# mike-gimelfarb/bboptpy

Hardware: AMD Instinct MI355X
Metric: candidate-evals/sec (higher is better)
Workload: dtype f64; 1 GPU; ActiveCMAES n=128 np=4096 rosenbrock, 256 independent populations per GPU in lockstep; populations_per_gpu=256, n=128, np=4096, objective=rosenbrock

## Files before the change

bboptpy_amd/csrc/bbo_cma.hip:

```cpp
#include "bbo_cma_kernels.hpp"
#include "bbo_sep_kernels.hpp"
#include "bbo_chol_kernels.hpp"
#include "bbo_eig_mw.hpp"

#include <algorithm>
#include <atomic>
#include <cmath>
#include <cstdlib>
#include <limits>

namespace bbo {

namespace {

enum { K_SAMPLE = 0, K_RANK, K_WHITEN, K_GRAM, K_PATHS, K_COV, K_EIGEN, K_POST, K_STOP, K_COUNT };
static const char *const K_NAMES[K_COUNT] = { "bbo:cma_sample_eval", "bbo:cma_rank", "bbo:cma_whiten", "bbo:cma_gram", "bbo:cma_paths", "bbo:cma_cov", "bbo:cma_eigen", "bbo:cma_post", "bbo:cma_history_stop" };

int pick_maxt(int ld)
{
    const int per_wave = ((ld >> 4) + 3) / 4;
    if (per_wave <= 1) return 1;
    if (per_wave <= 2) return 2;
    if (per_wave <= 4) return 4;
    return 8;
// ... 604 lines not shown
    return counter.fetch_add(1) & 7;
}

EigRoute CmaEngine::eig_route(bool spread_ok, bool fuse_ok) const
{
    const CmaConst &c = c_;
    const int dbg = d_.dbg;
    EigRoute r {};
    if (c.variant >= 2) return r;
    auto add = [&r](EigKernel k, int arg = 0) { r.step[r.count++] = EigRoute::Step { k, arg }; };
    const EigPlan pl_lds = eig_plan(c.n, c.ld);
    r.split = pl_lds.use_lds && pl_lds.threads == 512 && pl_lds.dc && c.npop <= split_maxp_
            && !(dbg & (DBG_QL | DBG_DC_NO_MERGES | DBG_DC_NO_LEAVES | DBG_TRED_L2 | DBG_EIG_ONE_WG));
    const EigPlan pl = r.split ? eig_plan_split(c.n, c.ld) : pl_lds;
    spread_ok = spread_ok && !mw_disabled_;
    const bool fixed_shape = c.n == 128 && c.ld == 128 && !d_.stamps
            && !(dbg & (DBG_EIG_IN_KERNEL | DBG_EIG_GENERIC128));
    bool big_spread = false, wy4_packs = false, fcols_closed = false;
    if (c.n <= 16 && c.n >= 2 && c.ld == 16 && !(dbg & DBG_NO_EIGEN_SMALL))
        add(EK_EIGEN_SMALL);
    else if (pl.threads < 512)
        add(pl.threads == 128 ? EK_EIGEN_128 : EK_EIGEN_256);
    else if (fixed_shape && c.npop > split_maxp_ && c.lazy_isc) {
        r.fixed = true;
        r.forms_c = fuse_ok && !(dbg & DBG_COV_UNFUSED);
        add(r.forms_c ? EK_EIGEN_FX128 : EK_EIGEN_FX128U);
    } else if (pl.use_lds)
        add(EK_EIGEN);
    else if (pl.hybrid && !(dbg & (DBG_QL | DBG_TRED_L2 | DBG_EIG_ONE_WG))) {
        if (r.split) {
            r.fixed = fixed_shape;
            add(r.fixed ? EK_EIGEN_R1_FX128 : EK_EIGEN_R1);
        } else if (spread_ok && !(dbg & DBG_TRED_ONE_WG)) {
            r.mw_workgroups = (long) c.npop * MW_G;
            const int istop = (dbg & DBG_TRED_ALL_SPREAD) ? 1 : 128;
            add(EK_TRED_MW, istop);
            if (istop > 1) add(EK_TRED_TAIL);
        } else
            add(EK_EIGEN_G1);
        add(EK_EIG_HALVES);
        if ((long) c.npop * 8 <= 256 && !(dbg & DBG_TOP_ONE_KERNEL)) {
// ... 58 lines not shown
    };
    timer_.begin(stream_, K_EIGEN);
    for (int i = 0; i < r.count; i++) {
        if (i == r.timed) {
            timer_.end(stream_);
            BBO_HIP(hipGetLastError());
        }
        const int arg = r.step[i].arg;
        switch (r.step[i].k) {
        case EK_EIGEN_SMALL:
            hipLaunchKernelGGL(cma_eigen_small, dim3((c.npop + 3) / 4), dim3(256), 0, stream_, d_, c_, 0, 1);
            break;
        case EK_EIGEN_128: per_matrix(cma_eigen_128, 128, pl, d_, c_, pl, 0); break;
        case EK_EIGEN_256: per_matrix(cma_eigen_256, 256, pl, d_, c_, pl, 0); break;
        case EK_EIGEN: per_matrix(cma_eigen, 512, pl, d_, c_, pl, 0); break;
        case EK_EIGEN_FX128: per_matrix(cma_eigen_fx128, 512, EIG_FX_PLAN, fa); break;
        case EK_EIGEN_FX128U: per_matrix(cma_eigen_fx128u, 512, EIG_FX_PLAN, fa); break;
        case EK_EIGEN_R1: per_matrix(cma_eigen_r1, 512, pl_lds, d_, c_, pl_lds, 0); break;
        case EK_EIGEN_R1_FX128: per_matrix(cma_eigen_r1_fx128, 512, EIG_FX_PLAN, fa); break;
        case EK_EIGEN_G1: per_matrix(cma_eigen_g1, 512, pl, d_, c_, pl, 0); break;
        case EK_TRED_MW:
            mw_launched_ = true;
            if (mw_buf_.count != (size_t) c.npop * MW_BUF_DOUBLES) mw_buf_.alloc((size_t) c.npop * MW_BUF_DOUBLES);
            hipLaunchKernelGGL(cma_tred_mw, dim3(8 * MW_G, c.npop), dim3(MW_T), 0, stream_, d_, c_, 0,
                    mw_buf_.p, ++mw_launch_, arg, mw_xcd_);
            break;
        case EK_TRED_TAIL: {
            const EigPlan plt = c.n > 256 ? eig_plan(256, 256) : pl;
            per_matrix(cma_tred_tail, 512, plt, d_, c_, plt, arg);
            break;
        }
        case EK_EIG_HALVES:
// ... 104 lines not shown
void CmaEngine::generation(bool honor_stop)
{
    if (small_fused_ok()) {
        launch_small(1, honor_stop);
        return;
    }
    small_fused_ = false;
    c_.honor_stop = honor_stop ? 1 : 0;
    launch_sample_eval();
    if (obj_.needs_host()) host_evaluate();
    else if (obj_.is_program()) program_evaluate();
    launch_rank();
    const EigRoute route = eig_route(true, true);
    launch_update(!route.forms_c);
    launch_eigen(route);
    launch_history_stop();
}

void CmaEngine::phase(int which)
{
    BBO_REQUIRE(inited_, "phase before init");
    BBO_HIP(hipSetDevice(params_.device));
    c_.honor_stop = 0;
    d_.mw_fault = mw_fault_from_env();
    switch (which) {
    case BBO_PHASE_SAMPLE_EVALUATE:
        launch_sample_eval();
        if (obj_.needs_host()) host_evaluate();
        else if (obj_.is_program()) program_evaluate();
        break;
    case BBO_PHASE_RANK: launch_rank(); break;
// ... 224 lines not shown
    if (k == "eig_stage") return o.one(s.eig_stage);
    if (k == "eig_mw_fail") return o.one(s.eig_mw_fail);
    if (k == "chol_repairs") {
        if (c.variant != 3) throw Error(BBO_ERR_KEY, "'chol_repairs' belongs to CholeskyCMAES");
        int r = 0;
        chol_repairs_.download(&r, 1, p);
        return o.one(r);
    }
    if (c.variant == 3 && k == "chol_tri") return o.one(chol_tri_ ? 1 : 0);
    if (c.variant == 3 && k == "stol") return o.one(c.stol);
    if (c.variant == 3 && k == "ranked") return o.one(c.ranked);
    if (k == "eig_mw_off") return o.one(mw_disabled_ ? 1 : 0);
    if (k == "eig_split_maxp") return o.one(split_maxp_);
    if (k == "eig_fixed128") return o.one(last_route_.fixed ? 1 : 0);
    if (k == "cov_fused") return o.one(last_route_.forms_c ? 1 : 0);
    if (k == "eig_route") {
        double ids[sizeof(last_route_.step) / sizeof(last_route_.step[0])];
        for (int i = 0; i < last_route_.count; i++) ids[i] = last_route_.step[i].k;
        return o.copy(ids, last_route_.count);
    }
    if (k == "rank_route") return o.one(last_rank_);
    if (k == "sample_route") return o.one(last_sample_.k);
    if (k == "sample_lean") return o.one(last_sample_.full);
    if (k == "update_route") {
        double ids[sizeof(last_update_.step) / sizeof(last_update_.step[0])];
        for (int i = 0; i < last_update_.count; i++) ids[i] = last_update_.step[i].k;
        return o.copy(ids, last_update_.count);
    }
    if (k == "small_fused") return o.one(small_fused_ ? 1 : 0);
    if (k == "splits") return o.one(c.splits);
// ... 187 lines not shown
```

bboptpy_amd/csrc/bbo_cma.hpp:

```cpp
#pragma once

#include "bbo_engine.hpp"

namespace bbo {

struct CmaScal {
    double sigma;
    double fbest, fworst;
    double pslen;
    double ybw[4];
    int ibw[4];
    int it, fev;
    int flag;
    int stop;
    int hsig;
    int eigenlastev, eigen_done;
    int hist_head, hist_len;
    int basis_ok;
    int eig_stage;
    int eig_mw_fail;
};

struct CmaConst {
    int n, ld;
// ... 35 lines not shown
    DBG_DC_LEAF16        = 32768,
    DBG_GRAM_NO_PACING   = 65536,
    DBG_PATHS_LAZY256    = 131072,
    DBG_RANK_BITONIC     = 262144,
    DBG_DC_LEAF_SINGLE   = 524288,
    DBG_SEP_ROWS_LDS     = 1048576,
    DBG_EIG_GENERIC128   = 2097152,
    DBG_EIG_ONE_WG       = 4194304,
    DBG_DC_WG_BARRIERS   = 8388608,
    DBG_TRED_ONE_WG      = 16777216,
    DBG_TOP_PART2        = 33554432,
    DBG_TOP_ONE_KERNEL   = 67108864,
    DBG_WY_PER_WAVE      = 134217728,
    DBG_SAMPLE_4WAVES    = 268435456,
    DBG_TRED_ALL_SPREAD  = 536870912,
    DBG_EIG_IN_KERNEL    = DBG_QL_NO_APPLY | DBG_QL | DBG_DC_NO_MERGES | DBG_DC_NO_LEAVES | DBG_TRED_L2
                           | DBG_STAMPS_HALVES | DBG_DC_ONE_LEVEL | DBG_DC_TWO_LEVELS | DBG_DC_LEAF16
                           | DBG_DC_LEAF_SINGLE | DBG_EIG_ONE_WG | DBG_DC_WG_BARRIERS,
};

struct CmaDev {
    double *X;
    double *f;
    int *rank;
    int *order;
    double *xmean, *xold, *pc, *ps;
    double *C;
    double *B;
    double *D;
    double *isc;
// ... 13 lines not shown
    const double *zinject;
    double *zrecord;
    CmaScal *scal;
    long long *stamps;
    int dbg;
    int mw_fault;
    int *mw_fail_host;
};

enum EigKernel : int {
    EK_EIGEN_SMALL = 0, EK_EIGEN_128, EK_EIGEN_256, EK_EIGEN, EK_EIGEN_FX128, EK_EIGEN_FX128U,
    EK_EIGEN_R1, EK_EIGEN_R1_FX128, EK_EIGEN_G1, EK_TRED_MW, EK_TRED_TAIL, EK_EIG_HALVES,
    EK_EIGEN_G2, EK_EIG_SECULAR, EK_EIG_LOWNER, EK_EIG_FCOLS, EK_EIGEN_G,
    EK_TRED_MW512, EK_TRED_MW_CHAIN, EK_EIGEN_B4, EK_EIGEN_B,
    EK_EIG_GEMM1, EK_EIG_GEMM, EK_EIG_WY4, EK_EIG_WY4_512, EK_EIG_WY,
    EK_POST, EK_POST_MFMA
};

struct EigRoute {
    struct Step {
        EigKernel k;
        int arg;
    };
    Step step[12];
    int count;
    int timed;
    bool split;
    bool post;
    bool fixed;
    bool forms_c;
    long mw_workgroups;
};

enum SampleKernel : int {
    SK_NONE = -1,
    SK_SEP_16 = 0, SK_SEP_64_512, SK_SEP_64_512_LEAN, SK_SEP_SUM, SK_SEP_SUM4, SK_SEP_64,
    SK_EVAL128, SK_EVAL128_TRI, SK_TILE8, SK_TILE8_TRI,
    SK_EVAL64_1_8, SK_EVAL64_1, SK_EVAL64_2,
    SK_TILE16, SK_EVAL_4, SK_EVAL_8
};

struct SampleRoute {
    SampleKernel k;
    int gx, gy, block;
    size_t lds;
// ... 114 lines not shown
```

bboptpy_amd/csrc/bbo_cma_kernels.hpp:

```cpp
#pragma once

#include "bbo_cma.hpp"
#include "bbo_objectives.hpp"
#include "bbo_rng.hpp"
#include "bbo_eig.hpp"
#include "bbo_rank.hpp"

namespace bbo {

typedef double d4_t __attribute__((ext_vector_type(4)));

#define BBO_INF (__builtin_huge_val())

__device__ inline void cma_draw_quad(const CmaDev &d, const CmaConst &c, int p, int row, int q,
        int gen, uint32_t sw, const double2 *tab, double (&z)[4])
{
    const int j0 = cma_quad_col0(q);
    z[0] = z[1] = z[2] = z[3] = 0.;
    if (row < c.lambda && j0 < c.n) {
        if (d.zinject) {
            const double *zi = d.zinject + ((size_t) p * c.lambda + row) * c.n;
#pragma unroll
            for (int i = 0; i < 4; i++)
                if (j0 + 4 * i < c.n) z[i] = zi[j0 + 4 * i];
// ... 1573 lines not shown
        const bool in = i < n && j < n;
        BDp[q] = in ? Bs[i * ldp + j] * Dv[j] : 0.;
    }
    if (mode == 2) {
        for (int q = q0 + tid; q < q1; q += 256) {
            const int t4 = q >> 6, l = q & 63;
            const int nt = t4 / KS, ks = t4 - nt * KS;
            const int i = nt * 16 + (l & 15), j = 4 * ks + (l >> 4);
            ISp[q] = (i < n && j < n) ? isc[(size_t) i * ld + j] : 0.;
        }
    }
}

__device__ __forceinline__ void history_stop_body(const CmaDev &d, const CmaConst &c, int p, int lane)
{
    CmaScal *sc = d.scal + p;
    if (pop_frozen(c, sc)) return;
    const int ld = c.ld, n = c.n;
    double *hb = d.hist_best + (size_t) p * c.hlen, *hk = d.hist_kth + (size_t) p * c.hlen;
    const double *f = d.f + (size_t) p * c.lambda_pad;
    const int *order = d.order + (size_t) p * c.lambda_pad;
    int it = sc->it;
    int head = sc->hist_head, len = sc->hist_len;
    double fbest = sc->fbest, fworst = sc->fworst;

    if (it < c.mit) {
        head = (head + 1) % c.hlen;
        if (lane == 0) {
            hb[head] = f[order[0]];
            hk[head] = f[order[c.ik]];
        }
        if (len < c.hlen) len++;
        wave_sync();
        if (len == c.hlen) {
            double lo = BBO_INF, hi = -BBO_INF;
            for (int k = lane; k < c.hlen; k += 64) {
                lo = fmin(lo, hb[k]);
                hi = fmax(hi, hb[k]);
            }
#pragma unroll
            for (int off = 32; off > 0; off >>= 1) {
                lo = fmin(lo, __shfl_xor(lo, off, 64));
                hi = fmax(hi, __shfl_xor(hi, off, 64));
            }
            fbest = lo;
            fworst = hi;
        }
    }
    it++;
    wave_sync();

    const double sigma = sc->sigma;
    const double *pc = d.pc + (size_t) p * ld, *xm = d.xmean + (size_t) p * ld;
    const double *C = d.C + (size_t) p * ld * ld, *B = d.B + (size_t) p * ld * ld;
    const double *D = d.D + (size_t) p * ld;
    int flag = 0;
    const int off = c.stop_off;
    if (it >= c.mit) {
        flag = 1;
    } else if (f[order[0]] <= c.ftarget) {
        flag = 10;
    } else if (!(off & 4) && it >= c.hlen && fworst - fbest < c.tol) {
        flag = 2;
    } else {
        if (!(off & 8) && len >= n) {
            int eq = 0;
            for (int i = lane; i < n; i += 64) {
                const int idx = (c.hlen + head - i) % c.hlen;
                eq += hb[idx] == hk[idx];
            }
#pragma unroll
            for (int off = 32; off > 0; off >>= 1) eq += __shfl_xor(eq, off, 64);
            if (3 * eq >= n) flag = 3;
        }
        const bool sep = c.variant == 2;
        if (!flag && !(off & 16)) {
            int bad = 0;
            for (int i = lane; i < n; i += 64) {
                const double sd = sep ? D[i] : sqrt(C[(size_t) i * ld + i]);
                bad |= (fmax(pc[i], sd) * sigma / c.sigma0 >= c.tol);
            }
            if (!__any(bad)) flag = 4;
        }
        if (!flag && !(off & 32) && sigma / c.sigma0 > 1.0e20 * D[n - 1]) flag = 5;
        if (!flag && !(off & 128) && D[n - 1] > 1.0e7 * D[0]) flag = 7;
        if (!flag && !(off & 256)) {
            const int iaxis = n - 1 - ((it - 1) % n);
            int moved = 0;
            if (sep) {
                moved = xm[iaxis] != xm[iaxis] + 0.1 * sigma * D[iaxis];
            } else {
                for (int i = lane; i < n; i += 64)
                    moved |= (xm[i] != xm[i] + 0.1 * sigma * D[iaxis] * B[(size_t) iaxis * ld + i]);
            }
            if (!__any(moved)) flag = 8;
        }
        if (!flag && !(off & 512)) {
            int stuck = 0;
            for (int i = lane; i < n; i += 64) {
                const double sd = sep ? D[i] : sqrt(C[(size_t) i * ld + i]);
                stuck |= (xm[i] == xm[i] + 0.2 * sigma * sd);
            }
            if (__any(stuck)) flag = 9;
        }
    }
    if (lane == 0) {
        sc->it = it;
        sc->hist_head = head;
        sc->hist_len = len;
        sc->fbest = fbest;
        sc->fworst = fworst;
        sc->flag = flag;
        if (flag) sc->stop = 1;
        else if (sc->fev >= c.mfev) sc->stop = 2;
    }
}

__global__ __launch_bounds__(64) void cma_history_stop(CmaDev d, CmaConst c)
{
    history_stop_body(d, c, blockIdx.x, threadIdx.x);
}

constexpr int SMALL_FUSED_MAXP = 512;

__host__ __device__ inline int small_state_doubles(const CmaConst &c)
{
    const int ld = c.ld, ld2 = ld * ld, lp = c.lambda_pad;
    return lp * ld
            + 2 * lp + lp
            + 5 * ld
// ... 228 lines not shown
```

bboptpy_amd/csrc/bbo_eig.hpp:

```cpp
#pragma once

#include <type_traits>

#include "bbo_cma.hpp"
#include "bbo_eig_ql.hpp"
#include "bbo_eig_dc.hpp"

namespace bbo {

typedef double d4_eig __attribute__((ext_vector_type(4)));

constexpr int EIG_THREADS = 512;
constexpr int EIG_NMAX = 512;

struct EigPlan {
    int threads;
    int use_lds;
    int reg_path;
    int dc;
    int hybrid;
    int lda;
    int rc;
    int vl;
    size_t lds_bytes;
// ... 149 lines not shown
    for (int a = 0; a < AMAX; a++)
#pragma unroll
        for (int b = 0; b < 8; b += 2) {
            acc0 = __builtin_fma(ur[a][b], a_[a][b], acc0);
            acc1 = __builtin_fma(ur[a][b + 1], a_[a][b + 1], acc1);
        }
    double acc = acc0 + acc1;
    acc = eig_quad_sum(acc);
    const double gq = -(acc / h);
#pragma unroll
    for (int a = 0; a < AMAX; a++)
#pragma unroll
        for (int b = 0; b < 8; b++) a_[a][b] = __builtin_fma(gq, ur[a][b], a_[a][b]);
}

template<int TT = EIG_THREADS>
__device__ inline void eig_tred_accum_reg128(const double *C, int ld, int n, const EigMat &As,
        double *dv, double *ev, double *uv, double *wv, double *gv, double *hvec, double *td,
        int tid, long long *stamps, double *qdst, int ldq, bool finish, bool accumulate = true)
{
    const int T = TT, lane = tid & 63;
    const int j = tid >> 2, q = tid & 3;
    double a_[4][8];
#pragma unroll
    for (int a = 0; a < 4; a++)
#pragma unroll
        for (int b = 0; b < 8; b++) {
            const int k = 32 * a + 8 * q + b;
            a_[a][b] = (j < n && k < n) ? C[(size_t) j * ld + k] : 0.;
        }
    for (int k = tid; k < 128; k += T) {
// ... 717 lines not shown
        wv[k] = 0.;
    }
    __syncthreads();
    const int lda = A.ld;
    for (int q = tid; q < n * n; q += T) {
        const int r = q / n, cidx = q - r * n;
        double v = 0.;
        if (cidx < r) v = r < 128 ? As(r, cidx) : A.a[(size_t) r * lda + cidx];
        Vout[q] = v;
    }
    __syncthreads();
    for (int k = tid; k < n; k += T) dv[k] = td[k];
    __syncthreads();
}

template<int TT>
__device__ inline void eig_cov_prologue128(const CmaDev &d, const CmaConst &c, const CmaScal *sc, int p,
        double *As, int tid)
{
    constexpr int N = 128, LB = eig_plan(128, 128).lda, EPT = 12;
    double *C = d.C + (size_t) p * N * N;
    const int lane = tid & 63, wave = __builtin_amdgcn_readfirstlane(tid >> 6);
    const double *pc = d.pc + (size_t) p * N;
    const int splits = c.splits;
    const double *G = d.gram_part + (size_t) p * splits * N * N;
    const CovCoef k = cov_coef(c, sc->hsig);
    const double pcl0 = pc[lane], pcl1 = pc[lane + 64];
    static_assert(24 % EPT == 0, "eig_cov_prologue128: 24 elements per thread");
#pragma unroll
    for (int e0 = 0; e0 < 24; e0 += EPT) {
        int off[EPT];
// ... 52 lines not shown
            double sum = cov_elem(k, cij[u], pci[u], h ? pcl1 : pcl0);
            sum += g[u];
            if (ok[u]) {
                As[i * LB + j] = sum;
                As[j * LB + i] = sum;
            }
        }
    }
    __syncthreads();
    for (int q = tid; q < N * (N / 2); q += TT) {
        const int r = q >> 6, c2 = (q & 63) * 2;
        *reinterpret_cast<double2*>(&C[r * N + c2]) = make_double2(As[r * LB + c2], As[r * LB + c2 + 1]);
    }
}

template<int TT, bool LDSM, int HYB = 1, int STAGE = 0, bool FX = false, bool PRO = false>
__device__ __forceinline__ void cma_eigen_impl(const CmaDev &d, const CmaConst &c, const EigPlan &pl,
        int force)
{
    const int p = blockIdx.x;
    CmaScal *sc = d.scal + p;
    if (c.honor_stop && sc->stop != 0) return;
    bool due = true;
    if (STAGE == 2 || STAGE == 4) {
        if (sc->eig_stage != 1) return;
    } else if (STAGE == 3) {
    } else
    if (!force && !((double) (sc->fev - sc->eigenlastev) > c.eigenfreq)) {
        if (threadIdx.x == 0) {
            sc->eigen_done = 0;
            sc->eig_stage = 0;
        }
        if (!PRO) return;
// ... 50 lines not shown
        }
        for (int r = wave; r < 128; r += T / 64)
            for (int cidx = lane; cidx < n; cidx += 64) Vout[(size_t) r * n + cidx] = cidx < r ? Ast(r, cidx) : 0.;
        if (tid == 0) sc->eig_stage = 1;
        return;
    }
    if (STAGE == 2 || STAGE == 4) {
        for (int i = tid; i < n; i += T) {
            dv[i] = STAGE == 2 ? tri[3 * n + i] : tri[i];
            ev[i] = tri[n + i];
            hvec[i] = tri[2 * n + i];
        }
        __syncthreads();
    } else {
    if (PRO) {
        eig_cov_prologue128<TT>(d, c, sc, p, A.a, tid);
        if (!due) return;
        eig_tred_accum_reg128<TT>(A.a, A.ld, n, A, dv, ev, uv, wv, gv, hvec, td, tid, nullptr, A.a, A.ld, true,
                !(pl.dc && !(d.dbg & DBG_QL)));
    } else if (LDSM) {
        eig_tred_accum_reg128<TT>(C, ld, n, A, dv, ev, uv, wv, gv, hvec, td, tid,
                (d.stamps && p == 0) ? d.stamps : nullptr, A.a, A.ld, true,
                !(pl.dc && !(d.dbg & DBG_QL)));
    } else if (TT == EIG_THREADS && !LDSM) {
        const bool hybrid = HYB != 0;
        EigMat Ast { reinterpret_cast<double*>(ibuf + 2 * EIG_MAXSEQ * 3 + 8), 128 };
        if (hybrid && !(d.dbg & DBG_QL) && !(d.dbg & DBG_TRED_L2))
            eig_tred_sym256(C, ld, n, A, dv, ev, uv, wv, gv, hvec, td, nv, tid,
                    (d.stamps && p == 0) ? d.stamps : nullptr, Ast, false,
                    d.eig_work + (size_t) (4 * p + 1) * eig_slab(ld));
        else
        eig_tred_accum_global(C, ld, n, A, dv, ev, uv, wv, gv, hvec, td, part, nv, tid,
                (d.stamps && p == 0) ? d.stamps : nullptr, hybrid ? &Ast : nullptr,
// ... 21 lines not shown
        if (tid == 0) {
            tri[4 * n] = 0.;
            sc->eig_stage = 1;
        }
        return;
    }

    const bool use_dc = pl.dc && !(d.dbg & DBG_QL);
    if (use_dc) {
        double *scr = uv;
        DcMat Qm { A.a, A.ld };
        double *Gp = d.eig_work + (size_t) (4 * p + 1) * eig_slab(ld);
        double *Bp_ = d.B + (size_t) p * ld * ld;
        long long *st_ = (d.stamps && p == 0 && !(STAGE == 2 && (d.dbg & DBG_STAMPS_HALVES))) ? d.stamps : nullptr;
        if (LDSM || HYB || TT != EIG_THREADS) {
            eig_dc_phase<TT, false, !LDSM, FX>(Qm, n, dv, ev, Gp, Bp_, ld, scr, st_, d.dbg, LDSM ? 0 : 1, hvec,
                    !LDSM && !(d.dbg & DBG_QL) && !(d.dbg & DBG_TRED_L2),
                    nullptr, STAGE == 2 ? 2 : 0, STAGE == 2 && tri[4 * n] != 0.,
                    STAGE == 2 ? force : 0, tri + 4 * n + 8);
            if (STAGE == 2 && force == 1) return;
        } else if (TT == EIG_THREADS && !LDSM) {
            eig_dc_phase<TT, true, true>(Qm, n, dv, ev, Gp, Bp_, ld, scr, st_, d.dbg, 1,
                    STAGE == 4 ? hvec : nullptr, STAGE == 4,
                    d.eig_work + (size_t) (4 * p + 3) * eig_slab(ld));
        }
    } else
    {
        QlState st { 0, 0, 1, 0, 0., 0., 0 };
        int prev_done = 0;
        for (int epoch = 0;; epoch++) {
            const int cur = epoch & 1;
// ... 71 lines not shown
    for (int i = tid; i < ld; i += T) Dp[i] = i < n ? sqrt(gv[i]) : 1.;
    if (!use_dc)
        for (int k = wave; k < n; k += T / 64)
            for (int j = lane; j < n; j += 64) Bp[(size_t) k * ld + perm[j]] = A(k, j);
    if (tid == 0) {
        sc->eigenlastev = sc->fev;
        sc->eigen_done = 1;
        sc->eig_stage = 0;
    }
    if (use_dc && LDSM && c.lazy_isc) {
        __syncthreads();
        for (int j = tid; j < n; j += T) dv[j] = sqrt(gv[j]);
        __syncthreads();
        double *BDp = d.BDp + (size_t) p * ld * ld;
        const int KS = ld >> 2;
        for (int q = tid; q < ld * ld; q += T) {
            const int t4 = q >> 6, l = q & 63;
            const int nt = t4 / KS, ks = t4 - nt * KS;
            const int i = nt * 16 + (l & 15), j = 4 * ks + (l >> 4);
            BDp[q] = (i < n && j < n) ? A(i, j) * dv[j] : 0.;
        }
        if (tid == 0) sc->basis_ok = 1;
    }
    EIG_STAMP(5);
#undef EIG_STAMP
}

__global__ __launch_bounds__(512) void cma_eigen(CmaDev d, CmaConst c, EigPlan pl, int force)
{
    cma_eigen_impl<512, true>(d, c, pl, force);
}
__global__ __launch_bounds__(512) void cma_eigen_g(CmaDev d, CmaConst c, EigPlan pl, int force)
{
    cma_eigen_impl<512, false, 1>(d, c, pl, force);
}
__global__ __launch_bounds__(512) void cma_eigen_b(CmaDev d, CmaConst c, EigPlan pl, int force)
{
    cma_eigen_impl<512, false, 0>(d, c, pl, force);
// ... 7 lines not shown
    const double *gram_part, *pc;
    double cc, c1, cmu, cneg, alphaold;
};
__device__ __forceinline__ void eig_fx_cov_args(const EigFxArgs &a, CmaDev &d, CmaConst &c)
{
    d.gram_part = const_cast<double*>(a.gram_part);
    d.pc = const_cast<double*>(a.pc);
    c.splits = a.splits;
    c.variant = a.variant;
    c.cc = a.cc;
    c.c1 = a.c1;
    c.cmu = a.cmu;
    c.cneg = a.cneg;
    c.alphaold = a.alphaold;
}
constexpr EigPlan EIG_FX_PLAN = eig_plan(128, 128);
template<bool PRO>
__device__ __forceinline__ void cma_eigen_fx128_body(const EigFxArgs &a)
{
    static_assert(EIG_FX_PLAN.use_lds == 1 && EIG_FX_PLAN.dc == 1 && EIG_FX_PLAN.reg_path == 1
            && EIG_FX_PLAN.threads == 512 && EIG_FX_PLAN.vl == 130, "cma_eigen_fx128: the plan of n = 128");
    CmaDev d {};
    d.C = a.C;
    d.B = a.B;
    d.D = a.D;
    d.BDp = a.BDp;
    d.eig_work = a.eig_work;
    d.scal = a.scal;
    CmaConst c {};
    c.n = c.ld = 128;
    c.lazy_isc = 1;
    c.honor_stop = a.honor_stop;
    c.eigenfreq = a.eigenfreq;
    if (PRO) eig_fx_cov_args(a, d, c);
    cma_eigen_impl<512, true, 1, 0, true, PRO>(d, c, EIG_FX_PLAN, 0);
}
__global__ __launch_bounds__(512) void cma_eigen_fx128(EigFxArgs a)
{
    cma_eigen_fx128_body<true>(a);
}
__global__ __launch_bounds__(512) void cma_eigen_fx128u(EigFxArgs a)
{
    cma_eigen_fx128_body<false>(a);
}
__global__ __launch_bounds__(512) void cma_eigen_r1_fx128(EigFxArgs a)
{
    CmaDev d {};
    d.C = a.C;
    d.eig_work = a.eig_work;
    d.scal = a.scal;
    CmaConst c {};
    c.n = c.ld = 128;
    c.honor_stop = a.honor_stop;
    c.eigenfreq = a.eigenfreq;
// ... 763 lines not shown
```

bboptpy_amd/csrc/bbo_eig_dc.hpp:

```cpp
#pragma once

#include <type_traits>

#include "bbo_cma.hpp"
#include "bbo_eig_ql.hpp"

namespace bbo {

typedef double dc_d4 __attribute__((ext_vector_type(4)));

constexpr int DC_LEAF = 16;
constexpr int DC_MAXB = 16;
constexpr int DC_MAXB_BIG = 32;
constexpr double DC_EPS = 0x1.0p-53;
constexpr int DC_KSTEPS = 32;

struct DcMat {
    double *a;
    int ld;
    __device__ double& operator()(int i, int j) const { return a[(size_t) i * ld + j]; }
};

__device__ inline void dc_sync(bool wv)
{
// ... 960 lines not shown
#pragma unroll
            for (int i = 0; i < 16; i++) {
                const double ti = i0 + i < n ? tau[i0 + i] : 0.;
                double sum = 0.;
#pragma unroll
                for (int m = 0; m < i; m++) sum = fma(t[m], Sb[m * LS + i], sum);
                t[i] = lane < i ? -ti * sum : (lane == i ? ti : 0.);
            }
#pragma unroll
            for (int i = 0; i < 16; i++) Tg[(size_t) b * 256 + lane * 16 + i] = t[i];
        }
        wave_sync();
    }
}

template<int TT>
__device__ inline void dc_apply_reflectors(const DcMat &Q, int n, const double *V, const double *tau,
        double *Tg, double *scratch, double *Bout, int ldb, const int *outpos,
        long long *stamps = nullptr, bool t_ready = false)
{
    const int tid = threadIdx.x, lane = tid & 63, wave = tid >> 6;
    const int fr = lane & 15, fk = lane >> 4;
    const int npanel = (n + 15) >> 4;
    constexpr int LDV = 132;
    const int outpos_col = (outpos && 16 * wave + fr < n) ? outpos[16 * wave + fr] : -1;
    __syncthreads();
    if (!t_ready) dc_build_T(n, V, tau, Tg, scratch);
    __threadfence_block();
    __syncthreads();
    if (stamps && threadIdx.x == 0) stamps[36] = wall_clock64();
    double *Vp = scratch;
// ... 79 lines not shown
        const int oc = outpos ? outpos_col : col;
#pragma unroll
        for (int rt = 0; rt < DC_KSTEPS / 4; rt++)
#pragma unroll
            for (int r = 0; r < 4; r++) {
                const int row = 16 * rt + fk + 4 * r;
                if (row < n) {
                    Bout[(size_t) row * ldb + oc] = qreg[rt][r];
                    Q(row, col) = qreg[rt][r];
                }
            }
    }
    __syncthreads();
}

template<int TT = 512, bool BIG = false, bool WIDE = true, bool FX = false>
__device__ __forceinline__ void eig_dc_phase(const DcMat &Q, int n_in, double *dv, double *ev, double *G,
        double *Bout, int ldb, double *scratch, long long *stamps_in, int dbg_in, int ext_top = 0,
        const double *hv = nullptr, bool qh_ready = false, double *Tscratch = nullptr, int mode = 0,
        bool t_prebuilt = false,
        int top_part = 0, double *Wimg = nullptr)
{
#define DC_STAMP(slot) do { if (stamps && threadIdx.x == 0) stamps[slot] = wall_clock64(); } while (0)
    static_assert(!FX || (TT == 512 && !BIG && !WIDE), "FX: the 512-thread kernel with the matrix in LDS");
    const int n = FX ? 128 : n_in, dbg = FX ? 0 : dbg_in;
    long long *const stamps = FX ? nullptr : stamps_in;
    DC_STAMP(16);
    const int tid = threadIdx.x, T = FX ? TT : blockDim.x, lane = tid & 63;
    const int wave = FX ? __builtin_amdgcn_readfirstlane(tid >> 6) : tid >> 6;
    const int NW = T >> 6;
    double *Qh = G;
    double *F = G + (size_t) n * n;
    constexpr int MAXB = BIG ? DC_MAXB_BIG : DC_MAXB;
    __shared__ int bounds[MAXB + 1];
    __shared__ int nblk_s;
    __shared__ int maxnr_s;
    __shared__ double scale_s;

    if (!qh_ready)
    for (int r = wave; r < n; r += NW)
        for (int c = lane; c < n; c += 64) Qh[(size_t) r * n + c] = Q(r, c);
// ... 81 lines not shown
            DcTeam tm;
            tm.id = wave / WPT;
            tm.active = 1;
            tm.wave0 = tm.id * WPT;
            tm.nwaves = WPT;
            tm.twave = wave & (WPT - 1);
            tm.ttid = tid - 64 * tm.wave0;
            tm.tthreads = 64 * WPT;
            tm.wave_scope = WPT == 1;
            tm.sorted_in = M > 16;
            if (tid == 0) maxnr_s = 0;
            __syncthreads();
            const int a = M * tm.id, mid = a + M / 2;
            dc_merge_level<4, true, false, WIDE, M>(Q, tm, a, mid, a + M, ev[mid - 1], dv, F + (size_t) a * n, W,
                    nullptr, M, nullptr);
        };
        level(std::integral_constant<int, 16>());
        level(std::integral_constant<int, 32>());
        level(std::integral_constant<int, 64>());
        level(std::integral_constant<int, 128>());
    }
    int nc = FX ? 1 : nblk;
    int levels_done = 0;
    while (nc > 1 && !(dbg & DBG_DC_NO_MERGES) && !((dbg & DBG_DC_ONE_LEVEL) && levels_done >= 1) && !((dbg & DBG_DC_TWO_LEVELS) && levels_done >= 2)) {
        const int L = levels_done;
        levels_done++;
        const int nm = nc >> 1;
        int teams = 1;
        while (teams < nm) teams <<= 1;
        int wpt = NW / teams > 0 ? NW / teams : 1;
// ... 79 lines not shown
    DC_STAMP(22);
    if (mode == 1) {
        for (int r = wave; r < n; r += NW)
            for (int cc = lane; cc < n; cc += 64) Bout[(size_t) r * ldb + (single ? W.outpos[cc] : cc)] = Q(r, cc);
        __syncthreads();
        return;
    }
    if (ext_top) {
        if (hv && !t_prebuilt) {
            __syncthreads();
            dc_build_T(n, Qh, taug, taug + n, scratch);
        }
        return;
    }
    if (hv) {
        dc_apply_reflectors<TT>(Q, n, Qh, taug, taug + n, scratch, Bout, ldb,
                single ? W.outpos : nullptr, stamps, t_early);
        DC_STAMP(23);
        return;
    }
    const int ntile = (n + 15) >> 4;
    const int ksteps = (n + 3) >> 2;
    const int fr = lane & 15, fk = lane >> 4;
    for (int rt = wave; rt < ntile; rt += NW) {
        double afrag[DC_KSTEPS];
        const int arow = rt * 16 + fr;
#pragma unroll
        for (int ks = 0; ks < DC_KSTEPS; ks++) {
            const int kk = 4 * ks + fk;
            afrag[ks] = (arow < n && kk < n) ? Qh[(size_t) arow * n + kk] : 0.;
        }
// ... 26 lines not shown
```

Before: 723.3 million candidate-evals/s.

## Fold history/stop tests into the fixed-shape 128 eigen kernel

The separate history_stop kernel launch for the n=128 fixed eigen route is removed. The stop tests now run on wave 0 inside cma_eigen_fx128, in the BD-packing loop or on the early-return path when no eigendecomposition is due, while the other waves take over the packing loop. The aim is to cut one kernel launch and its global reloads per generation, at the cost of fewer threads doing the packing store. A separate stamped (CLK) variant is also added for profiling with timestamps.

```diff
diff --git a/bboptpy_amd/csrc/bbo_cma.hip b/bboptpy_amd/csrc/bbo_cma.hip
--- a/bboptpy_amd/csrc/bbo_cma.hip
+++ b/bboptpy_amd/csrc/bbo_cma.hip
@@ -642,8 +642,8 @@
             && !(dbg & (DBG_QL | DBG_DC_NO_MERGES | DBG_DC_NO_LEAVES | DBG_TRED_L2 | DBG_EIG_ONE_WG));
     const EigPlan pl = r.split ? eig_plan_split(c.n, c.ld) : pl_lds;
     spread_ok = spread_ok && !mw_disabled_;
-    const bool fixed_shape = c.n == 128 && c.ld == 128 && !d_.stamps
-            && !(dbg & (DBG_EIG_IN_KERNEL | DBG_EIG_GENERIC128));
+    const bool fx_shape = c.n == 128 && c.ld == 128 && !(dbg & (DBG_EIG_IN_KERNEL | DBG_EIG_GENERIC128));
+    const bool fixed_shape = fx_shape && !d_.stamps;
     bool big_spread = false, wy4_packs = false, fcols_closed = false;
     if (c.n <= 16 && c.n >= 2 && c.ld == 16 && !(dbg & DBG_NO_EIGEN_SMALL))
         add(EK_EIGEN_SMALL);
@@ -652,7 +652,12 @@
     else if (fixed_shape && c.npop > split_maxp_ && c.lazy_isc) {
         r.fixed = true;
         r.forms_c = fuse_ok && !(dbg & DBG_COV_UNFUSED);
-        add(r.forms_c ? EK_EIGEN_FX128 : EK_EIGEN_FX128U);
+        r.runs_stop = r.forms_c && !(dbg & DBG_STOP_UNFOLDED);
+        add(r.runs_stop ? EK_EIGEN_FX128 : r.forms_c ? EK_EIGEN_FX128C : EK_EIGEN_FX128U);
+    } else if (fx_shape && d_.stamps && fuse_ok && !(dbg & DBG_COV_UNFUSED) && c.npop > split_maxp_ && c.lazy_isc) {
+        r.fixed = true;
+        r.forms_c = true;
+        add(EK_EIGEN_FX128_CLK);
     } else if (pl.use_lds)
         add(EK_EIGEN);
     else if (pl.hybrid && !(dbg & (DBG_QL | DBG_TRED_L2 | DBG_EIG_ONE_WG))) {
@@ -741,8 +746,14 @@
         case EK_EIGEN_128: per_matrix(cma_eigen_128, 128, pl, d_, c_, pl, 0); break;
         case EK_EIGEN_256: per_matrix(cma_eigen_256, 256, pl, d_, c_, pl, 0); break;
         case EK_EIGEN: per_matrix(cma_eigen, 512, pl, d_, c_, pl, 0); break;
-        case EK_EIGEN_FX128: per_matrix(cma_eigen_fx128, 512, EIG_FX_PLAN, fa); break;
+        case EK_EIGEN_FX128:
+            per_matrix(cma_eigen_fx128, 512, EIG_FX_PLAN, EigFxFoldArgs { fa, EigFxStopArgs { d_.hist_best, d_.hist_kth,
+                    d_.f, d_.order, d_.xmean, c.ftarget, c.tol, c.sigma0, c.lambda_pad, c.hlen, c.mit, c.ik, c.mfev,
+                    c.stop_off } });
+            break;
+        case EK_EIGEN_FX128C: per_matrix(cma_eigen_fx128c, 512, EIG_FX_PLAN, fa); break;
         case EK_EIGEN_FX128U: per_matrix(cma_eigen_fx128u, 512, EIG_FX_PLAN, fa); break;
+        case EK_EIGEN_FX128_CLK: per_matrix(cma_eigen_fx128_clk, 512, EIG_FX_PLAN, EigFxClkArgs { fa, d_.stamps }); break;
         case EK_EIGEN_R1: per_matrix(cma_eigen_r1, 512, pl_lds, d_, c_, pl_lds, 0); break;
         case EK_EIGEN_R1_FX128: per_matrix(cma_eigen_r1_fx128, 512, EIG_FX_PLAN, fa); break;
         case EK_EIGEN_G1: per_matrix(cma_eigen_g1, 512, pl, d_, c_, pl, 0); break;
@@ -877,7 +888,7 @@
     const EigRoute route = eig_route(true, true);
     launch_update(!route.forms_c);
     launch_eigen(route);
-    launch_history_stop();
+    if (!last_route_.runs_stop) launch_history_stop();
 }
 
 void CmaEngine::phase(int which)
@@ -1132,6 +1143,7 @@
     if (k == "eig_split_maxp") return o.one(split_maxp_);
     if (k == "eig_fixed128") return o.one(last_route_.fixed ? 1 : 0);
     if (k == "cov_fused") return o.one(last_route_.forms_c ? 1 : 0);
+    if (k == "stop_fused") return o.one(last_route_.runs_stop ? 1 : 0);
     if (k == "eig_route") {
         double ids[sizeof(last_route_.step) / sizeof(last_route_.step[0])];
         for (int i = 0; i < last_route_.count; i++) ids[i] = last_route_.step[i].k;
diff --git a/bboptpy_amd/csrc/bbo_cma.hpp b/bboptpy_amd/csrc/bbo_cma.hpp
--- a/bboptpy_amd/csrc/bbo_cma.hpp
+++ b/bboptpy_amd/csrc/bbo_cma.hpp
@@ -73,6 +73,7 @@
     DBG_WY_PER_WAVE      = 134217728,
     DBG_SAMPLE_4WAVES    = 268435456,
     DBG_TRED_ALL_SPREAD  = 536870912,
+    DBG_STOP_UNFOLDED    = 1073741824,
     DBG_EIG_IN_KERNEL    = DBG_QL_NO_APPLY | DBG_QL | DBG_DC_NO_MERGES | DBG_DC_NO_LEAVES | DBG_TRED_L2
                            | DBG_STAMPS_HALVES | DBG_DC_ONE_LEVEL | DBG_DC_TWO_LEVELS | DBG_DC_LEAF16
                            | DBG_DC_LEAF_SINGLE | DBG_EIG_ONE_WG | DBG_DC_WG_BARRIERS,
@@ -116,7 +117,8 @@
     EK_EIGEN_G2, EK_EIG_SECULAR, EK_EIG_LOWNER, EK_EIG_FCOLS, EK_EIGEN_G,
     EK_TRED_MW512, EK_TRED_MW_CHAIN, EK_EIGEN_B4, EK_EIGEN_B,
     EK_EIG_GEMM1, EK_EIG_GEMM, EK_EIG_WY4, EK_EIG_WY4_512, EK_EIG_WY,
-    EK_POST, EK_POST_MFMA
+    EK_POST, EK_POST_MFMA,
+    EK_EIGEN_FX128_CLK, EK_EIGEN_FX128C
 };
 
 struct EigRoute {
@@ -131,6 +133,7 @@
     bool post;
     bool fixed;
     bool forms_c;
+    bool runs_stop;
     long mw_workgroups;
 };
 
diff --git a/bboptpy_amd/csrc/bbo_cma_kernels.hpp b/bboptpy_amd/csrc/bbo_cma_kernels.hpp
--- a/bboptpy_amd/csrc/bbo_cma_kernels.hpp
+++ b/bboptpy_amd/csrc/bbo_cma_kernels.hpp
@@ -1611,106 +1611,7 @@
 
 __device__ __forceinline__ void history_stop_body(const CmaDev &d, const CmaConst &c, int p, int lane)
 {
-    CmaScal *sc = d.scal + p;
-    if (pop_frozen(c, sc)) return;
-    const int ld = c.ld, n = c.n;
-    double *hb = d.hist_best + (size_t) p * c.hlen, *hk = d.hist_kth + (size_t) p * c.hlen;
-    const double *f = d.f + (size_t) p * c.lambda_pad;
-    const int *order = d.order + (size_t) p * c.lambda_pad;
-    int it = sc->it;
-    int head = sc->hist_head, len = sc->hist_len;
-    double fbest = sc->fbest, fworst = sc->fworst;
-
-    if (it < c.mit) {
-        head = (head + 1) % c.hlen;
-        if (lane == 0) {
-            hb[head] = f[order[0]];
-            hk[head] = f[order[c.ik]];
-        }
-        if (len < c.hlen) len++;
-        wave_sync();
-        if (len == c.hlen) {
-            double lo = BBO_INF, hi = -BBO_INF;
-            for (int k = lane; k < c.hlen; k += 64) {
-                lo = fmin(lo, hb[k]);
-                hi = fmax(hi, hb[k]);
-            }
-#pragma unroll
-            for (int off = 32; off > 0; off >>= 1) {
-                lo = fmin(lo, __shfl_xor(lo, off, 64));
-                hi = fmax(hi, __shfl_xor(hi, off, 64));
-            }
-            fbest = lo;
-            fworst = hi;
-        }
-    }
-    it++;
-    wave_sync();
-
-    const double sigma = sc->sigma;
-    const double *pc = d.pc + (size_t) p * ld, *xm = d.xmean + (size_t) p * ld;
-    const double *C = d.C + (size_t) p * ld * ld, *B = d.B + (size_t) p * ld * ld;
-    const double *D = d.D + (size_t) p * ld;
-    int flag = 0;
-    const int off = c.stop_off;
-    if (it >= c.mit) {
-        flag = 1;
-    } else if (f[order[0]] <= c.ftarget) {
-        flag = 10;
-    } else if (!(off & 4) && it >= c.hlen && fworst - fbest < c.tol) {
-        flag = 2;
-    } else {
-        if (!(off & 8) && len >= n) {
-            int eq = 0;
-            for (int i = lane; i < n; i += 64) {
-                const int idx = (c.hlen + head - i) % c.hlen;
-                eq += hb[idx] == hk[idx];
-            }
-#pragma unroll
-            for (int off = 32; off > 0; off >>= 1) eq += __shfl_xor(eq, off, 64);
-            if (3 * eq >= n) flag = 3;
-        }
-        const bool sep = c.variant == 2;
-        if (!flag && !(off & 16)) {
-            int bad = 0;
-            for (int i = lane; i < n; i += 64) {
-                const double sd = sep ? D[i] : sqrt(C[(size_t) i * ld + i]);
-                bad |= (fmax(pc[i], sd) * sigma / c.sigma0 >= c.tol);
-            }
-            if (!__any(bad)) flag = 4;
-        }
-        if (!flag && !(off & 32) && sigma / c.sigma0 > 1.0e20 * D[n - 1]) flag = 5;
-        if (!flag && !(off & 128) && D[n - 1] > 1.0e7 * D[0]) flag = 7;
-        if (!flag && !(off & 256)) {
-            const int iaxis = n - 1 - ((it - 1) % n);
-            int moved = 0;
-            if (sep) {
-                moved = xm[iaxis] != xm[iaxis] + 0.1 * sigma * D[iaxis];
-            } else {
-                for (int i = lane; i < n; i += 64)
-                    moved |= (xm[i] != xm[i] + 0.1 * sigma * D[iaxis] * B[(size_t) iaxis * ld + i]);
-            }
-            if (!__any(moved)) flag = 8;
-        }
-        if (!flag && !(off & 512)) {
-            int stuck = 0;
-            for (int i = lane; i < n; i += 64) {
-                const double sd = sep ? D[i] : sqrt(C[(size_t) i * ld + i]);
-                stuck |= (xm[i] == xm[i] + 0.2 * sigma * sd);
-            }
-            if (__any(stuck)) flag = 9;
-        }
-    }
-    if (lane == 0) {
-        sc->it = it;
-        sc->hist_head = head;
-        sc->hist_len = len;
-        sc->fbest = fbest;
-        sc->fworst = fworst;
-        sc->flag = flag;
-        if (flag) sc->stop = 1;
-        else if (sc->fev >= c.mfev) sc->stop = 2;
-    }
+    history_stop_view(stop_view(d, c), p, lane);
 }
 
 __global__ __launch_bounds__(64) void cma_history_stop(CmaDev d, CmaConst c)
diff --git a/bboptpy_amd/csrc/bbo_cma_stop.hpp b/bboptpy_amd/csrc/bbo_cma_stop.hpp
--- /dev/null
+++ b/bboptpy_amd/csrc/bbo_cma_stop.hpp
@@ -0,0 +1,130 @@
+#pragma once
+
+#include "bbo_cma.hpp"
+#include "bbo_wave.hpp"
+
+namespace bbo {
+
+struct StopView {
+    CmaScal *scal;
+    double *hist_best, *hist_kth;
+    const double *f;
+    const int *order;
+    const double *pc, *xmean;
+    const double *C, *B, *D;
+    double ftarget, tol, sigma0;
+    int n, ld, lambda_pad, hlen, mit, ik, mfev, stop_off, variant, honor_stop;
+};
+
+__device__ __forceinline__ StopView stop_view(const CmaDev &d, const CmaConst &c)
+{
+    return StopView { d.scal, d.hist_best, d.hist_kth, d.f, d.order, d.pc, d.xmean, d.C, d.B, d.D,
+            c.ftarget, c.tol, c.sigma0, c.n, c.ld, c.lambda_pad, c.hlen, c.mit, c.ik, c.mfev, c.stop_off,
+            c.variant, c.honor_stop };
+}
+
+__device__ __forceinline__ void history_stop_view(const StopView &c, int p, int lane)
+{
+    CmaScal *sc = c.scal + p;
+    if (pop_frozen(c, sc)) return;
+    const int ld = c.ld, n = c.n;
+    double *hb = c.hist_best + (size_t) p * c.hlen, *hk = c.hist_kth + (size_t) p * c.hlen;
+    const double *f = c.f + (size_t) p * c.lambda_pad;
+    const int *order = c.order + (size_t) p * c.lambda_pad;
+    int it = sc->it;
+    int head = sc->hist_head, len = sc->hist_len;
+    double fbest = sc->fbest, fworst = sc->fworst;
+
+    if (it < c.mit) {
+        head = (head + 1) % c.hlen;
+        if (lane == 0) {
+            hb[head] = f[order[0]];
+            hk[head] = f[order[c.ik]];
+        }
+        if (len < c.hlen) len++;
+        wave_sync();
+        if (len == c.hlen) {
+            double lo = __builtin_huge_val(), hi = -__builtin_huge_val();
+            for (int k = lane; k < c.hlen; k += 64) {
+                lo = fmin(lo, hb[k]);
+                hi = fmax(hi, hb[k]);
+            }
+#pragma unroll
+            for (int off = 32; off > 0; off >>= 1) {
+                lo = fmin(lo, __shfl_xor(lo, off, 64));
+                hi = fmax(hi, __shfl_xor(hi, off, 64));
+            }
+            fbest = lo;
+            fworst = hi;
+        }
+    }
+    it++;
+    wave_sync();
+
+    const double sigma = sc->sigma;
+    const double *pc = c.pc + (size_t) p * ld, *xm = c.xmean + (size_t) p * ld;
+    const double *C = c.C + (size_t) p * ld * ld, *B = c.B + (size_t) p * ld * ld;
+    const double *D = c.D + (size_t) p * ld;
+    int flag = 0;
+    const int off = c.stop_off;
+    if (it >= c.mit) {
+        flag = 1;
+    } else if (f[order[0]] <= c.ftarget) {
+        flag = 10;
+    } else if (!(off & 4) && it >= c.hlen && fworst - fbest < c.tol) {
+        flag = 2;
+    } else {
+        if (!(off & 8) && len >= n) {
+            int eq = 0;
+            for (int i = lane; i < n; i += 64) {
+                const int idx = (c.hlen + head - i) % c.hlen;
+                eq += hb[idx] == hk[idx];
+            }
+#pragma unroll
+            for (int off = 32; off > 0; off >>= 1) eq += __shfl_xor(eq, off, 64);
+            if (3 * eq >= n) flag = 3;
+        }
+        const bool sep = c.variant == 2;
+        if (!flag && !(off & 16)) {
+            int bad = 0;
+            for (int i = lane; i < n; i += 64) {
+                const double sd = sep ? D[i] : sqrt(C[(size_t) i * ld + i]);
+                bad |= (fmax(pc[i], sd) * sigma / c.sigma0 >= c.tol);
+            }
+            if (!__any(bad)) flag = 4;
+        }
+        if (!flag && !(off & 32) && sigma / c.sigma0 > 1.0e20 * D[n - 1]) flag = 5;
+        if (!flag && !(off & 128) && D[n - 1] > 1.0e7 * D[0]) flag = 7;
+        if (!flag && !(off & 256)) {
+            const int iaxis = n - 1 - ((it - 1) % n);
+            int moved = 0;
+            if (sep) {
+                moved = xm[iaxis] != xm[iaxis] + 0.1 * sigma * D[iaxis];
+            } else {
+                for (int i = lane; i < n; i += 64)
+                    moved |= (xm[i] != xm[i] + 0.1 * sigma * D[iaxis] * B[(size_t) iaxis * ld + i]);
+            }
+            if (!__any(moved)) flag = 8;
+        }
+        if (!flag && !(off & 512)) {
+            int stuck = 0;
+            for (int i = lane; i < n; i += 64) {
+                const double sd = sep ? D[i] : sqrt(C[(size_t) i * ld + i]);
+                stuck |= (xm[i] == xm[i] + 0.2 * sigma * sd);
+            }
+            if (__any(stuck)) flag = 9;
+        }
+    }
+    if (lane == 0) {
+        sc->it = it;
+        sc->hist_head = head;
+        sc->hist_len = len;
+        sc->fbest = fbest;
+        sc->fworst = fworst;
+        sc->flag = flag;
+        if (flag) sc->stop = 1;
+        else if (sc->fev >= c.mfev) sc->stop = 2;
+    }
+}
+
+}
diff --git a/bboptpy_amd/csrc/bbo_eig.hpp b/bboptpy_amd/csrc/bbo_eig.hpp
--- a/bboptpy_amd/csrc/bbo_eig.hpp
+++ b/bboptpy_amd/csrc/bbo_eig.hpp
@@ -3,6 +3,7 @@
 #include <type_traits>
 
 #include "bbo_cma.hpp"
+#include "bbo_cma_stop.hpp"
 #include "bbo_eig_ql.hpp"
 #include "bbo_eig_dc.hpp"
 
@@ -187,7 +188,7 @@
         for (int b = 0; b < 8; b++) a_[a][b] = __builtin_fma(gq, ur[a][b], a_[a][b]);
 }
 
-template<int TT = EIG_THREADS>
+template<int TT = EIG_THREADS, bool OWN = false>
 __device__ inline void eig_tred_accum_reg128(const double *C, int ld, int n, const EigMat &As,
         double *dv, double *ev, double *uv, double *wv, double *gv, double *hvec, double *td,
         int tid, long long *stamps, double *qdst, int ldq, bool finish, bool accumulate = true)
@@ -935,7 +936,7 @@
     __syncthreads();
 }
 
-template<int TT>
+template<int TT, bool OWN = false>
 __device__ inline void eig_cov_prologue128(const CmaDev &d, const CmaConst &c, const CmaScal *sc, int p,
         double *As, int tid)
 {
@@ -1018,9 +1019,13 @@
     }
 }
 
-template<int TT, bool LDSM, int HYB = 1, int STAGE = 0, bool FX = false, bool PRO = false>
+struct EigFxFoldArgs;
+typedef const __attribute__((address_space(4))) EigFxFoldArgs *EigFxKernarg;
+__device__ __forceinline__ void eig_fx_stop_tests(EigFxKernarg ka, int p, int tid);
+template<int TT, bool LDSM, int HYB = 1, int STAGE = 0, bool FX = false, bool PRO = false, bool CLK = false,
+        bool FOLD = false>
 __device__ __forceinline__ void cma_eigen_impl(const CmaDev &d, const CmaConst &c, const EigPlan &pl,
-        int force)
+        int force, EigFxKernarg ka = nullptr)
 {
     const int p = blockIdx.x;
     CmaScal *sc = d.scal + p;
@@ -1101,9 +1106,20 @@
         __syncthreads();
     } else {
     if (PRO) {
-        eig_cov_prologue128<TT>(d, c, sc, p, A.a, tid);
-        if (!due) return;
-        eig_tred_accum_reg128<TT>(A.a, A.ld, n, A, dv, ev, uv, wv, gv, hvec, td, tid, nullptr, A.a, A.ld, true,
+        eig_cov_prologue128<TT, CLK>(d, c, sc, p, A.a, tid);
+        if (!due) {
+            if (FOLD) {
+                __syncthreads();
+                if (tid < 64) eig_fx_stop_tests(ka, p, tid);
+            }
+            return;
+        }
+        if (CLK) {
+            __syncthreads();
+            EIG_STAMP(6);
+        }
+        eig_tred_accum_reg128<TT, CLK>(A.a, A.ld, n, A, dv, ev, uv, wv, gv, hvec, td, tid,
+                (CLK && d.stamps && p == 0) ? d.stamps : nullptr, A.a, A.ld, true,
                 !(pl.dc && !(d.dbg & DBG_QL)));
     } else if (LDSM) {
         eig_tred_accum_reg128<TT>(C, ld, n, A, dv, ev, uv, wv, gv, hvec, td, tid,
@@ -1155,7 +1171,7 @@
         double *Bp_ = d.B + (size_t) p * ld * ld;
         long long *st_ = (d.stamps && p == 0 && !(STAGE == 2 && (d.dbg & DBG_STAMPS_HALVES))) ? d.stamps : nullptr;
         if (LDSM || HYB || TT != EIG_THREADS) {
-            eig_dc_phase<TT, false, !LDSM, FX>(Qm, n, dv, ev, Gp, Bp_, ld, scr, st_, d.dbg, LDSM ? 0 : 1, hvec,
+            eig_dc_phase<TT, false, !LDSM, FX, CLK>(Qm, n, dv, ev, Gp, Bp_, ld, scr, st_, d.dbg, LDSM ? 0 : 1, hvec,
                     !LDSM && !(d.dbg & DBG_QL) && !(d.dbg & DBG_TRED_L2),
                     nullptr, STAGE == 2 ? 2 : 0, STAGE == 2 && tri[4 * n] != 0.,
                     STAGE == 2 ? force : 0, tri + 4 * n + 8);
@@ -1257,7 +1273,10 @@
         __syncthreads();
         double *BDp = d.BDp + (size_t) p * ld * ld;
         const int KS = ld >> 2;
-        for (int q = tid; q < ld * ld; q += T) {
+        if (FOLD && tid < 64) {
+            eig_fx_stop_tests(ka, p, tid);
+        } else
+        for (int q = FOLD ? tid - 64 : tid; q < ld * ld; q += FOLD ? T - 64 : T) {
             const int t4 = q >> 6, l = q & 63;
             const int nt = t4 / KS, ks = t4 - nt * KS;
             const int i = nt * 16 + (l & 15), j = 4 * ks + (l >> 4);
@@ -1265,6 +1284,7 @@
         }
         if (tid == 0) sc->basis_ok = 1;
     }
+    if (CLK) __syncthreads();
     EIG_STAMP(5);
 #undef EIG_STAMP
 }
@@ -1302,9 +1322,28 @@
     c.cneg = a.cneg;
     c.alphaold = a.alphaold;
 }
+struct EigFxStopArgs {
+    double *hist_best, *hist_kth;
+    const double *f;
+    const int *order;
+    const double *xmean;
+    double ftarget, tol, sigma0;
+    int lambda_pad, hlen, mit, ik, mfev, stop_off;
+};
+struct EigFxFoldArgs {
+    EigFxArgs a;
+    EigFxStopArgs s;
+};
+__device__ __forceinline__ void eig_fx_stop_tests(EigFxKernarg ka, int p, int tid)
+{
+    const StopView v { ka->a.scal, ka->s.hist_best, ka->s.hist_kth, ka->s.f, ka->s.order, ka->a.pc, ka->s.xmean,
+            ka->a.C, ka->a.B, ka->a.D, ka->s.ftarget, ka->s.tol, ka->s.sigma0, 128, 128, ka->s.lambda_pad,
+            ka->s.hlen, ka->s.mit, ka->s.ik, ka->s.mfev, ka->s.stop_off, 0, ka->a.honor_stop };
+    history_stop_view(v, p, tid);
+}
 constexpr EigPlan EIG_FX_PLAN = eig_plan(128, 128);
-template<bool PRO>
-__device__ __forceinline__ void cma_eigen_fx128_body(const EigFxArgs &a)
+template<bool PRO, bool CLK = false, bool FOLD = false>
+__device__ __forceinline__ void cma_eigen_fx128_body(const EigFxArgs &a, long long *stamps = nullptr)
 {
     static_assert(EIG_FX_PLAN.use_lds == 1 && EIG_FX_PLAN.dc == 1 && EIG_FX_PLAN.reg_path == 1
             && EIG_FX_PLAN.threads == 512 && EIG_FX_PLAN.vl == 130, "cma_eigen_fx128: the plan of n = 128");
@@ -1321,11 +1360,25 @@
     c.honor_stop = a.honor_stop;
     c.eigenfreq = a.eigenfreq;
     if (PRO) eig_fx_cov_args(a, d, c);
-    cma_eigen_impl<512, true, 1, 0, true, PRO>(d, c, EIG_FX_PLAN, 0);
-}
-__global__ __launch_bounds__(512) void cma_eigen_fx128(EigFxArgs a)
+    if (CLK) d.stamps = stamps;
+    cma_eigen_impl<512, true, 1, 0, true, PRO, CLK, FOLD>(d, c, EIG_FX_PLAN, 0,
+            FOLD ? (EigFxKernarg) __builtin_amdgcn_kernarg_segment_ptr() : nullptr);
+}
+__global__ __launch_bounds__(512) void cma_eigen_fx128(EigFxFoldArgs fa)
+{
+    cma_eigen_fx128_body<true, false, true>(fa.a);
+}
+__global__ __launch_bounds__(512) void cma_eigen_fx128c(EigFxArgs a)
 {
     cma_eigen_fx128_body<true>(a);
+}
+struct EigFxClkArgs {
+    EigFxArgs a;
+    long long *stamps;
+};
+__global__ __launch_bounds__(512) void cma_eigen_fx128_clk(EigFxClkArgs ca)
+{
+    cma_eigen_fx128_body<true, true>(ca.a, ca.stamps);
 }
 __global__ __launch_bounds__(512) void cma_eigen_fx128u(EigFxArgs a)
 {
diff --git a/bboptpy_amd/csrc/bbo_eig_dc.hpp b/bboptpy_amd/csrc/bbo_eig_dc.hpp
--- a/bboptpy_amd/csrc/bbo_eig_dc.hpp
+++ b/bboptpy_amd/csrc/bbo_eig_dc.hpp
@@ -998,7 +998,7 @@
     }
 }
 
-template<int TT>
+template<int TT, bool OWN = false>
 __device__ inline void dc_apply_reflectors(const DcMat &Q, int n, const double *V, const double *tau,
         double *Tg, double *scratch, double *Bout, int ldb, const int *outpos,
         long long *stamps = nullptr, bool t_ready = false)
@@ -1108,7 +1108,7 @@
     __syncthreads();
 }
 
-template<int TT = 512, bool BIG = false, bool WIDE = true, bool FX = false>
+template<int TT = 512, bool BIG = false, bool WIDE = true, bool FX = false, bool CLK = false>
 __device__ __forceinline__ void eig_dc_phase(const DcMat &Q, int n_in, double *dv, double *ev, double *G,
         double *Bout, int ldb, double *scratch, long long *stamps_in, int dbg_in, int ext_top = 0,
         const double *hv = nullptr, bool qh_ready = false, double *Tscratch = nullptr, int mode = 0,
@@ -1118,7 +1118,7 @@
 #define DC_STAMP(slot) do { if (stamps && threadIdx.x == 0) stamps[slot] = wall_clock64(); } while (0)
     static_assert(!FX || (TT == 512 && !BIG && !WIDE), "FX: the 512-thread kernel with the matrix in LDS");
     const int n = FX ? 128 : n_in, dbg = FX ? 0 : dbg_in;
-    long long *const stamps = FX ? nullptr : stamps_in;
+    long long *const stamps = (FX && !CLK) ? nullptr : stamps_in;
     DC_STAMP(16);
     const int tid = threadIdx.x, T = FX ? TT : blockDim.x, lane = tid & 63;
     const int wave = FX ? __builtin_amdgcn_readfirstlane(tid >> 6) : tid >> 6;
@@ -1230,6 +1230,10 @@
             const int a = M * tm.id, mid = a + M / 2;
             dc_merge_level<4, true, false, WIDE, M>(Q, tm, a, mid, a + M, ev[mid - 1], dv, F + (size_t) a * n, W,
                     nullptr, M, nullptr);
+            if (CLK) {
+                __syncthreads();
+                DC_STAMP(M == 16 ? 24 : M == 32 ? 25 : M == 64 ? 26 : 27);
+            }
         };
         level(std::integral_constant<int, 16>());
         level(std::integral_constant<int, 32>());
@@ -1339,7 +1343,7 @@
         return;
     }
     if (hv) {
-        dc_apply_reflectors<TT>(Q, n, Qh, taug, taug + n, scratch, Bout, ldb,
+        dc_apply_reflectors<TT, CLK>(Q, n, Qh, taug, taug + n, scratch, Bout, ldb,
                 single ? W.outpos : nullptr, stamps, t_early);
         DC_STAMP(23);
         return;
```

New measurement: 727.6 million candidate-evals/s, median of 6. About the same (+0.6%).
